# faustomorales/keras-ocr

Hardware: AMD Instinct MI355X
Metric: images/sec end-to-end Pipeline.recognize() @768x768 (higher is better)
Workload: dtype f32 (fp32 operands as 2 fp16 pieces [F(4,3) / head layers] or 3 bf16 pieces [1x1, dilated], 3 / 6 MFMA products, fp32 accumulate; fp32-class error vs fp64: tests/test_conv_gpu.py)

## Files before the change

keras_ocr_amd/csrc/elementwise.hip:

```cpp
#include "split_common.h"
#include <algorithm>

struct EwParams {
  const float* in;
  float* out;
  int N, Hi, Wi, Ho, Wo, C4;
  int in_cs, in_co, out_cs, out_co;
  float sy, sx;
  int row_off;
  int Wov;
};

__global__ void maxpool2x2_kernel(EwParams p) {
  const size_t total = (size_t)p.N * p.Ho * p.Wo * p.C4;
  for (size_t i = blockIdx.x * (size_t)blockDim.x + threadIdx.x; i < total;
       i += (size_t)gridDim.x * blockDim.x) {
    const int c4 = i % p.C4;
    size_t t = i / p.C4;
    const int ox = t % p.Wo;
    t /= p.Wo;
    const int oy = t % p.Ho;
    const int n = t / p.Ho;
    const size_t o = (((size_t)n * p.Ho + oy) * p.Wo + ox) * p.out_cs + p.out_co + c4 * 4;
    if (ox >= p.Wov) {
      *reinterpret_cast<float4*>(p.out + o) = float4{0.f, 0.f, 0.f, 0.f};
      continue;
    }
    const size_t base = (((size_t)n * p.Hi + 2 * oy + p.row_off) * p.Wi + 2 * ox) * p.in_cs + p.in_co + c4 * 4;
    const float4 a = *reinterpret_cast<const float4*>(p.in + base);
    const float4 b = *reinterpret_cast<const float4*>(p.in + base + p.in_cs);
    const float4 c = *reinterpret_cast<const float4*>(p.in + base + (size_t)p.Wi * p.in_cs);
    const float4 d = *reinterpret_cast<const float4*>(p.in + base + (size_t)p.Wi * p.in_cs + p.in_cs);
    float4 r;
    r.x = fmaxf(fmaxf(a.x, b.x), fmaxf(c.x, d.x));
    r.y = fmaxf(fmaxf(a.y, b.y), fmaxf(c.y, d.y));
    r.z = fmaxf(fmaxf(a.z, b.z), fmaxf(c.z, d.z));
    r.w = fmaxf(fmaxf(a.w, b.w), fmaxf(c.w, d.w));
    *reinterpret_cast<float4*>(p.out + o) = r;
  }
}

__global__ void maxpool3x3s1_kernel(EwParams p) {
  const size_t total = (size_t)p.N * p.Ho * p.Wo * p.C4;
  for (size_t i = blockIdx.x * (size_t)blockDim.x + threadIdx.x; i < total;
       i += (size_t)gridDim.x * blockDim.x) {
    const int c4 = i % p.C4;
    size_t t = i / p.C4;
    const int ox = t % p.Wo;
    t /= p.Wo;
    const int oy = t % p.Ho;
    const int n = t / p.Ho;
    float4 r = make_float4(-INFINITY, -INFINITY, -INFINITY, -INFINITY);
    for (int dy = -1; dy <= 1; ++dy) {
      const int iy = oy + dy;
      if (iy < 0 || iy >= p.Hi) continue;
      for (int dx = -1; dx <= 1; ++dx) {
        const int ix = ox + dx;
        if (ix < 0 || ix >= p.Wi) continue;
        const float4 v = *reinterpret_cast<const float4*>(
            p.in + (((size_t)n * p.Hi + iy) * p.Wi + ix) * p.in_cs + p.in_co + c4 * 4);
        r.x = fmaxf(r.x, v.x);
        r.y = fmaxf(r.y, v.y);
        r.z = fmaxf(r.z, v.z);
        r.w = fmaxf(r.w, v.w);
      }
    }
    const size_t o = (((size_t)n * p.Ho + oy) * p.Wo + ox) * p.out_cs + p.out_co + c4 * 4;
    *reinterpret_cast<float4*>(p.out + o) = r;
  }
}

__global__ void resize_bilinear_kernel(EwParams p) {
  const size_t total = (size_t)p.N * p.Ho * p.Wo * p.C4;
  for (size_t i = blockIdx.x * (size_t)blockDim.x + threadIdx.x; i < total;
       i += (size_t)gridDim.x * blockDim.x) {
    const int c4 = i % p.C4;
    size_t t = i / p.C4;
    const int ox = t % p.Wo;
    t /= p.Wo;
    const int oy = t % p.Ho;
    const int n = t / p.Ho;
    const float fy = ((float)oy + 0.5f) * p.sy - 0.5f;
    const float fx = ((float)ox + 0.5f) * p.sx - 0.5f;
    const float fly = floorf(fy), flx = floorf(fx);
    const int y0 = max((int)fly, 0), y1 = min((int)ceilf(fy), p.Hi - 1);
    const int x0 = max((int)flx, 0), x1 = min((int)ceilf(fx), p.Wi - 1);
    const float yl = fy - fly, xl = fx - flx, yk = 1.f - yl, xk = 1.f - xl;
    const size_t rb = (size_t)n * p.Hi;
    const float* b0 = p.in + ((rb + y0) * p.Wi) * p.in_cs + p.in_co + c4 * 4;
    const float* b1 = p.in + ((rb + y1) * p.Wi) * p.in_cs + p.in_co + c4 * 4;
    const float4 tl = *reinterpret_cast<const float4*>(b0 + (size_t)x0 * p.in_cs);
    const float4 tr = *reinterpret_cast<const float4*>(b0 + (size_t)x1 * p.in_cs);
    const float4 bl = *reinterpret_cast<const float4*>(b1 + (size_t)x0 * p.in_cs);
    const float4 br = *reinterpret_cast<const float4*>(b1 + (size_t)x1 * p.in_cs);
    float4 r;
    {
      const float top = tl.x * xk + tr.x * xl, bot = bl.x * xk + br.x * xl;
      r.x = top * yk + bot * yl;
    }
    {
      const float top = tl.y * xk + tr.y * xl, bot = bl.y * xk + br.y * xl;
      r.y = top * yk + bot * yl;
    }
    {
      const float top = tl.z * xk + tr.z * xl, bot = bl.z * xk + br.z * xl;
      r.z = top * yk + bot * yl;
    }
    {
      const float top = tl.w * xk + tr.w * xl, bot = bl.w * xk + br.w * xl;
      r.w = top * yk + bot * yl;
    }
    const size_t o = (((size_t)n * p.Ho + oy) * p.Wo + ox) * p.out_cs + p.out_co + c4 * 4;
    *reinterpret_cast<float4*>(p.out + o) = r;
  }
}

__global__ void copy_channels_kernel(EwParams p) {
  const size_t total = (size_t)p.N * p.Ho * p.Wo * p.C4;
  for (size_t i = blockIdx.x * (size_t)blockDim.x + threadIdx.x; i < total;
       i += (size_t)gridDim.x * blockDim.x) {
    const int c4 = i % p.C4;
    const size_t px = i / p.C4;
    *reinterpret_cast<float4*>(p.out + px * p.out_cs + p.out_co + c4 * 4) =
        *reinterpret_cast<const float4*>(p.in + px * p.in_cs + p.in_co + c4 * 4);
  }
}

static int check_vec(kocr_ctx* ctx, const Tensor& in, const Tensor& out, const char* what) {
  if (in.C != out.C || in.N != out.N) KOCR_FAIL(ctx, KOCR_EINVAL, std::string(what) + ": shape mismatch");
  if (in.C % 4 || in.cs % 4 || in.co % 4 || out.cs % 4 || out.co % 4)
    KOCR_FAIL(ctx, KOCR_EINVAL, std::string(what) + ": channels must be multiples of 4");
  return KOCR_OK;
}

static EwParams make_params(const Tensor& in, const Tensor& out) {
  EwParams p;
  p.in = in.p;
  p.out = out.p;
  p.N = in.N;
  p.Hi = in.H;
  p.Wi = in.W;
  p.Ho = out.H;
  p.Wo = out.W;
  p.C4 = in.C / 4;
  p.in_cs = in.cs;
  p.in_co = in.co;
  p.out_cs = out.cs;
  p.out_co = out.co;
  p.sy = p.sx = 1.f;
  p.row_off = 0;
  p.Wov = out.W;
  return p;
}

static dim3 ew_grid(size_t total) {
  size_t b = (total + 255) / 256;
  if (b > 256 * 16) b = 256 * 16;
  if (b == 0) b = 1;
  return dim3((unsigned)b);
}

int launch_maxpool2x2(kocr_ctx* ctx, const Tensor& in, const Tensor& out, int row_off) {
  KOCR_TRY(check_vec(ctx, in, out, "maxpool2x2"));
  if (out.H != (in.H - row_off) / 2 || out.wv() != in.wv() / 2) KOCR_FAIL(ctx, KOCR_EINVAL, "maxpool2x2: bad output size");
  EwParams p = make_params(in, out);
  p.row_off = row_off;
  p.Wov = out.wv();
  const size_t total = out.pixels() * p.C4;
  if (!total) return KOCR_OK;
  {
    ProfScope ps(ctx, "maxpool2x2", 0, 4.0 * (in.pixels() + out.pixels()) * in.C);
    hipLaunchKernelGGL(maxpool2x2_kernel, ew_grid(total), dim3(256), 0, ctx->stream, p);
    KOCR_HIP(ctx, hipGetLastError());
  }
  if (out.amax) {
    if (in.amax) return launch_amax_copy(ctx, in.amax, out.amax, out.N);
    return launch_absmax(ctx, out, out.amax);
  }
  return KOCR_OK;
}

int launch_maxpool3x3s1(kocr_ctx* ctx, const Tensor& in, const Tensor& out) {
  KOCR_TRY(check_vec(ctx, in, out, "maxpool3x3s1"));
  if (out.H != in.H || out.W != in.W) KOCR_FAIL(ctx, KOCR_EINVAL, "maxpool3x3s1: bad output size");
  EwParams p = make_params(in, out);
  const size_t total = out.pixels() * p.C4;
  if (!total) return KOCR_OK;
  {
    ProfScope ps(ctx, "maxpool3x3s1", 0, 4.0 * (in.pixels() + out.pixels()) * in.C);
    hipLaunchKernelGGL(maxpool3x3s1_kernel, ew_grid(total), dim3(256), 0, ctx->stream, p);
    KOCR_HIP(ctx, hipGetLastError());
  }
  if (out.amax) {
    if (in.amax) return launch_amax_copy(ctx, in.amax, out.amax, out.N);
    return launch_absmax(ctx, out, out.amax);
  }
  return KOCR_OK;
}

int launch_resize_bilinear(kocr_ctx* ctx, const Tensor& in, const Tensor& out) {
  KOCR_TRY(check_vec(ctx, in, out, "resize_bilinear"));
  EwParams p = make_params(in, out);
  p.sy = (float)in.H / (float)out.H;
  p.sx = (float)in.W / (float)out.W;
  const size_t total = out.pixels() * p.C4;
  if (!total) return KOCR_OK;
  {
    ProfScope ps(ctx, "resize_bilinear", 0, 4.0 * (in.pixels() + out.pixels()) * in.C);
    hipLaunchKernelGGL(resize_bilinear_kernel, ew_grid(total), dim3(256), 0, ctx->stream, p);
    KOCR_HIP(ctx, hipGetLastError());
  }
  if (out.amax) {
    if (in.amax) return launch_amax_copy(ctx, in.amax, out.amax, out.N);
    return launch_absmax(ctx, out, out.amax);
  }
  return KOCR_OK;
}

int launch_copy_channels(kocr_ctx* ctx, const Tensor& in, const Tensor& out) {
  KOCR_TRY(check_vec(ctx, in, out, "copy_channels"));
  if (out.H != in.H || out.W != in.W) KOCR_FAIL(ctx, KOCR_EINVAL, "copy_channels: bad output size");
  EwParams p = make_params(in, out);
  const size_t total = out.pixels() * p.C4;
  if (!total) return KOCR_OK;
  ProfScope ps(ctx, "copy_channels", 0, 8.0 * out.pixels() * in.C);
  hipLaunchKernelGGL(copy_channels_kernel, ew_grid(total), dim3(256), 0, ctx->stream, p);
  KOCR_HIP(ctx, hipGetLastError());
  return KOCR_OK;
}

struct HeadTailParams {
  const float* in;
  float* out;
  const float* w6;
  const float* a6;
  const float* b6;
  const float* w8;
  const float* a8;
  const float* b8;
  int ld6, ld8, in_cs, in_co, relu6;
  size_t P;
};

__global__ __launch_bounds__(256) void head_tail_kernel(HeadTailParams p) {
  __shared__ float s_w6[16][16], s_a6[16], s_b6[16], s_w8[16][2], s_a8[2], s_b8[2];
  const int tid = threadIdx.x;
  s_w6[tid >> 4][tid & 15] = p.w6[(tid >> 4) * p.ld6 + (tid & 15)];
  if (tid < 16) {
    s_a6[tid] = p.a6[tid];
    s_b6[tid] = p.b6[tid];
    s_w8[tid][0] = p.w8[tid * p.ld8 + 0];
    s_w8[tid][1] = p.w8[tid * p.ld8 + 1];
  }
  if (tid < 2) {
    s_a8[tid] = p.a8[tid];
    s_b8[tid] = p.b8[tid];
  }
  __syncthreads();
  typedef float v4f __attribute__((ext_vector_type(4)));
  typedef float v2f __attribute__((ext_vector_type(2)));
  for (size_t i = blockIdx.x * (size_t)blockDim.x + tid; i < p.P; i += (size_t)gridDim.x * blockDim.x) {
    const float* src = p.in + i * p.in_cs + p.in_co;
    float x[16];
#pragma unroll
    for (int q = 0; q < 4; ++q) {
      const v4f v = *reinterpret_cast<const v4f*>(src + 4 * q);
      x[4 * q + 0] = v.x;
      x[4 * q + 1] = v.y;
      x[4 * q + 2] = v.z;
      x[4 * q + 3] = v.w;
    }
    float y0 = 0.f, y1 = 0.f;
#pragma unroll
    for (int o = 0; o < 16; ++o) {
      float h = 0.f;
#pragma unroll
      for (int c = 0; c < 16; ++c) h = fmaf(x[c], s_w6[c][o], h);
      h = h * s_a6[o] + s_b6[o];
      if (p.relu6) h = fmaxf(h, 0.f);
      y0 = fmaf(h, s_w8[o][0], y0);
      y1 = fmaf(h, s_w8[o][1], y1);
    }
    *reinterpret_cast<v2f*>(p.out + 2 * i) = v2f{y0 * s_a8[0] + s_b8[0], y1 * s_a8[1] + s_b8[1]};
  }
}

int launch_head_tail(kocr_ctx* ctx, const ConvLayer& L6, const ConvLayer& L8, const Tensor& in, float* d_heat) {
  if (L6.Cin != 16 || L6.Cout != 16 || L6.KH != 1 || L8.Cin != 16 || L8.Cout != 2 || L8.KH != 1 || L8.relu ||
      L6.d_post_a || L8.d_post_a || !L6.tap_inner || !L8.tap_inner || in.C != 16 || in.cs % 4 || in.co % 4)
    KOCR_FAIL(ctx, KOCR_EINVAL, "head_tail: unexpected layer shapes");
  HeadTailParams p;
  p.in = in.p;
  p.out = d_heat;
  p.w6 = L6.d_w;
  p.a6 = L6.d_pre_a;
  p.b6 = L6.d_pre_b;
  p.w8 = L8.d_w;
  p.a8 = L8.d_pre_a;
  p.b8 = L8.d_pre_b;
  p.ld6 = L6.Cout_pad;
  p.ld8 = L8.Cout_pad;
  p.in_cs = in.cs;
  p.in_co = in.co;
  p.relu6 = L6.relu;
  p.P = in.pixels();
  if (!p.P) return KOCR_OK;
  const double flops = 2.0 * (double)p.P * (16 * 16 + 16 * 2);
  ProfScope ps(ctx, "conv_head_tail", flops, (double)p.P * (64 + 8));
  hipLaunchKernelGGL(head_tail_kernel, ew_grid(p.P), dim3(256), 0, ctx->stream, p);
  KOCR_HIP(ctx, hipGetLastError());
  return KOCR_OK;
}

__global__ __launch_bounds__(256) void absmax_kernel(const float* in, size_t img_pixels, int C4, int cs, int co, unsigned* slots) {
  typedef float v4f __attribute__((ext_vector_type(4)));
  float m = 0.f;
  const size_t total = img_pixels * C4;
  const float* base = in + (size_t)blockIdx.y * img_pixels * cs;
  for (size_t i = blockIdx.x * (size_t)blockDim.x + threadIdx.x; i < total; i += (size_t)gridDim.x * blockDim.x) {
    const size_t px = i / C4;
    const int c4 = (int)(i - px * C4);
    const v4f v = *reinterpret_cast<const v4f*>(base + px * cs + co + 4 * c4);
    m = fmaxf(m, fmaxf(fmaxf(fabsf(v.x), fabsf(v.y)), fmaxf(fabsf(v.z), fabsf(v.w))));
  }
  kocr_amax_update(slots + blockIdx.y, m);
}

__global__ void amax_copy_kernel(const unsigned* from, unsigned* to, int n) {
  const int i = blockIdx.x * blockDim.x + threadIdx.x;
  if (i < n) atomicMax(to + i, from[i]);
}

int launch_absmax(kocr_ctx* ctx, const Tensor& t, unsigned* slots) {
  if (t.C % 4 || t.cs % 4 || t.co % 4 || ((uintptr_t)t.p & 15)) KOCR_FAIL(ctx, KOCR_EINVAL, "absmax: unaligned tensor");
  const size_t total = (size_t)t.H * t.W * (t.C / 4);
  if (!total || !t.N) return KOCR_OK;
  ProfScope ps(ctx, "absmax", 0, 4.0 * t.pixels() * t.C);
  size_t b = (total + 4095) / 4096;
  const size_t cap = std::max<size_t>(1, 4096 / (size_t)t.N);
  if (b > cap) b = cap;
  constexpr int NCHUNK = 32768;
  for (int n0 = 0; n0 < t.N; n0 += NCHUNK) {
    const int nn = std::min(NCHUNK, t.N - n0);
    hipLaunchKernelGGL(absmax_kernel, dim3((unsigned)b, (unsigned)nn), dim3(256), 0, ctx->stream,
                       t.p + (size_t)n0 * t.H * t.W * t.cs, (size_t)t.H * t.W, t.C / 4, t.cs, t.co, slots + n0);
    KOCR_HIP(ctx, hipGetLastError());
  }
  return KOCR_OK;
}

__global__ __launch_bounds__(256) void range_stats_kernel(const float* in, int H, int W, int C4, int cs, int co, const unsigned* slots,
                                                          int cells, int cellW, int top, unsigned long long* cnt, double* sums, int n0) {
  typedef float v4f __attribute__((ext_vector_type(4)));
  const int n = n0 + blockIdx.y;
  const size_t img_pixels = (size_t)H * W, total = img_pixels * C4;
  const float* base = in + (size_t)n * img_pixels * cs;
  unsigned long long c0 = 0, c1 = 0, c2 = 0;
  double s0 = 0, s1 = 0;
  for (size_t i = blockIdx.x * (size_t)blockDim.x + threadIdx.x; i < total; i += (size_t)gridDim.x * blockDim.x) {
    const size_t px = i / C4;
    const int c4 = (int)(i - px * C4);
    const int slot = cells ? n * cells + (int)((px % W) / cellW) : n;
    const int e = kocr_scale_exp(slots + slot, top);
    const float sc = kocr_pow2(e);
    const v4f v = *reinterpret_cast<const v4f*>(base + px * cs + co + 4 * c4);
#pragma unroll
    for (int k = 0; k < 4; ++k) {
      const float a = fabsf(v[k]), s = a * sc;
      if (a > 0.f) {
        ++c0;
        s0 += a;
        if (s < 0.0625f) {
          ++c1;
          s1 += a;
        }
        if (s < 6.103515625e-05f) ++c2;
      }
    }
  }
  atomicAdd(cnt + 0, c0);
  atomicAdd(cnt + 1, c1);
  atomicAdd(cnt + 2, c2);
  atomicAdd(sums + 0, s0);
  atomicAdd(sums + 1, s1);
}

int launch_range_stats(kocr_ctx* ctx, const std::string& name, const Tensor& t, const unsigned* slots, int top) {
  if (!ctx->range_on || !slots || t.C % 4 || t.cs % 4 || t.co % 4 || !t.pixels()) return KOCR_OK;
  if (!ctx->d_range) KOCR_FAIL(ctx, KOCR_EINVAL, "range statistics: call kocr_range_stats_enable first");
  unsigned long long* cnt = (unsigned long long*)ctx->d_range;
  double* sums = (double*)((char*)ctx->d_range + 32);
  KOCR_HIP(ctx, hipMemsetAsync(ctx->d_range, 0, 64, ctx->stream));
  size_t b = ((size_t)t.H * t.W * (t.C / 4) + 4095) / 4096;
  if (b > 64) b = 64;
  constexpr int NCHUNK = 32768;
  for (int n0 = 0; n0 < t.N; n0 += NCHUNK) {
    hipLaunchKernelGGL(range_stats_kernel, dim3((unsigned)b, (unsigned)std::min(NCHUNK, t.N - n0)), dim3(256), 0, ctx->stream, t.p, t.H,
                       t.W, t.C / 4, t.cs, t.co, slots, t.cells(), t.cellW ? t.cellW : 1, top, cnt, sums, n0);
    KOCR_HIP(ctx, hipGetLastError());
  }
  unsigned long long hc[4];
  double hs[4];
  KOCR_HIP(ctx, hipMemcpyAsync(hc, cnt, 32, hipMemcpyDeviceToHost, ctx->stream));
  KOCR_HIP(ctx, hipMemcpyAsync(hs, sums, 32, hipMemcpyDeviceToHost, ctx->stream));
  KOCR_HIP(ctx, hipStreamSynchronize(ctx->stream));
  RangeRow& r = ctx->range[name];
  r.launches += 1;
  r.elements += (double)t.pixels() * t.C;
  r.nonzero += (double)hc[0];
  r.below_m4 += (double)hc[1];
  r.below_m14 += (double)hc[2];
  r.sum_abs += hs[0];
  r.sum_abs_below_m4 += hs[1];
  return KOCR_OK;
}

int launch_amax_copy(kocr_ctx* ctx, const unsigned* from, unsigned* to, int n) {
  if (!from || !to || from == to || n <= 0) return KOCR_OK;
  hipLaunchKernelGGL(amax_copy_kernel, dim3((n + 255) / 256), dim3(256), 0, ctx->stream, from, to, n);
  KOCR_HIP(ctx, hipGetLastError());
  return KOCR_OK;
}
```

keras_ocr_amd/csrc/imgproc.hip:

```cpp
#include "common.h"
#include <cmath>

struct ResizeTables {
  int* xi0;
  int* xi1;
  int* xa0;
  int* xa1;
  int* yi0;
  int* yi1;
  int* yb0;
  int* yb1;
};

namespace {
void axis_tables(int src, int dst, bool horizontal, std::vector<int>& i0, std::vector<int>& i1, std::vector<int>& c0,
                 std::vector<int>& c1) {
  const double scale = (double)src / (double)dst;
  i0.resize(dst);
  i1.resize(dst);
  c0.resize(dst);
  c1.resize(dst);
  for (int d = 0; d < dst; ++d) {
    float f = (float)((d + 0.5) * scale - 0.5);
    int s = (int)std::floor(f);
    f = f - (float)s;
    if (horizontal) {
      if (s < 0) {
        f = 0.f;
        s = 0;
      }
      if (s >= src - 1) {
        f = 0.f;
        s = src - 1;
      }
    }
    c1[d] = (int)std::nearbyint(f * 2048.f);
    c0[d] = (int)std::nearbyint((1.f - f) * 2048.f);
    i0[d] = std::min(std::max(s, 0), src - 1);
    i1[d] = std::min(std::max(s + 1, 0), src - 1);
  }
}
}

__global__ void resize_pad_kernel(const uint8_t* __restrict__ src, int sh, int sw, size_t src_img_stride,
                                  uint8_t* __restrict__ dst, int dh, int dw, int Hmax, int Wmax, int cval, ResizeTables t) {
  const int n = blockIdx.z, y = blockIdx.y;
  const int x = blockIdx.x * blockDim.x + threadIdx.x;
  if (x >= Wmax) return;
  uint8_t* o = dst + (((size_t)n * Hmax + y) * Wmax + x) * 3;
  if (y >= dh || x >= dw) {
    o[0] = o[1] = o[2] = (uint8_t)cval;
    return;
  }
  const uint8_t* im = src + (size_t)n * src_img_stride;
  const int x0 = t.xi0[x], x1 = t.xi1[x], a0 = t.xa0[x], a1 = t.xa1[x];
  const int y0 = t.yi0[y], y1 = t.yi1[y], b0 = t.yb0[y], b1 = t.yb1[y];
  const uint8_t* r0 = im + (size_t)y0 * sw * 3;
  const uint8_t* r1 = im + (size_t)y1 * sw * 3;
#pragma unroll
  for (int c = 0; c < 3; ++c) {
    const int S0 = r0[x0 * 3 + c] * a0 + r0[x1 * 3 + c] * a1;
    const int S1 = r1[x0 * 3 + c] * a0 + r1[x1 * 3 + c] * a1;
    const int v = (((b0 * (S0 >> 4)) >> 16) + ((b1 * (S1 >> 4)) >> 16) + 2) >> 2;
    o[c] = (uint8_t)min(max(v, 0), 255);
  }
}

int launch_resize_pad(kocr_ctx* ctx, const uint8_t* d_src, int n, int sh, int sw, uint8_t* d_dst, int dh, int dw,
                      int Hmax, int Wmax, int cval, Arena& tab_arena) {
  if (n <= 0) return KOCR_OK;
  if (dh <= 0 || dw <= 0 || dh > Hmax || dw > Wmax || sh <= 0 || sw <= 0)
    KOCR_FAIL(ctx, KOCR_EINVAL, "resize_pad: bad sizes");
  std::vector<int> tb[8];
  axis_tables(sw, dw, true, tb[0], tb[1], tb[2], tb[3]);
  axis_tables(sh, dh, false, tb[4], tb[5], tb[6], tb[7]);
  std::vector<int> flat;
  for (auto& v : tb) flat.insert(flat.end(), v.begin(), v.end());
  int* d_tab = (int*)arena_alloc(tab_arena, flat.size() * sizeof(int));
  if (!d_tab) KOCR_FAIL(ctx, KOCR_ENOMEM, "resize_pad: table arena exhausted");
  KOCR_HIP(ctx, hipMemcpyAsync(d_tab, flat.data(), flat.size() * sizeof(int), hipMemcpyHostToDevice, ctx->stream));
  KOCR_HIP(ctx, hipStreamSynchronize(ctx->stream));
  ResizeTables t;
  t.xi0 = d_tab;
  t.xi1 = t.xi0 + dw;
  t.xa0 = t.xi1 + dw;
  t.xa1 = t.xa0 + dw;
  t.yi0 = t.xa1 + dw;
  t.yi1 = t.yi0 + dh;
  t.yb0 = t.yi1 + dh;
  t.yb1 = t.yb0 + dh;
  ProfScope ps(ctx, "resize_pad", 0, 3.0 * n * ((double)sh * sw + (double)Hmax * Wmax));
  hipLaunchKernelGGL(resize_pad_kernel, dim3((Wmax + 255) / 256, Hmax, n), dim3(256), 0, ctx->stream, d_src, sh, sw,
                     (size_t)sh * sw * 3, d_dst, dh, dw, Hmax, Wmax, cval, t);
  KOCR_HIP(ctx, hipGetLastError());
  return KOCR_OK;
}


struct ResizeTablesF {
  int* xi0;
  int* xi1;
  float* xa;
  int* yi0;
  int* yi1;
  float* ya;
};

__global__ void resize_pad_f32_kernel(const float* __restrict__ src, int sh, int sw, int C, float* __restrict__ dst, int dh, int dw,
                                      int Hmax, int Wmax, float cval, ResizeTablesF t) {
  const int n = blockIdx.z, y = blockIdx.y;
  const int x = blockIdx.x * blockDim.x + threadIdx.x;
  if (x >= Wmax) return;
  float* o = dst + (((size_t)n * Hmax + y) * Wmax + x) * C;
  if (y >= dh || x >= dw) {
    for (int c = 0; c < C; ++c) o[c] = cval;
    return;
  }
  const float* im = src + (size_t)n * sh * sw * C;
  const int x0 = t.xi0[x], x1 = t.xi1[x], y0 = t.yi0[y], y1 = t.yi1[y];
  const float ax = t.xa[x], ay = t.ya[y];
  const float* r0 = im + (size_t)y0 * sw * C;
  const float* r1 = im + (size_t)y1 * sw * C;
  for (int c = 0; c < C; ++c) {
    const float h0 = r0[x0 * C + c] * (1.f - ax) + r0[x1 * C + c] * ax;
    const float h1 = r1[x0 * C + c] * (1.f - ax) + r1[x1 * C + c] * ax;
    o[c] = h0 * (1.f - ay) + h1 * ay;
  }
}

int launch_resize_pad_f32(kocr_ctx* ctx, const float* d_src, int n, int sh, int sw, int C, float* d_dst, int dh, int dw, int Hmax,
                          int Wmax, float cval, Arena& tab_arena) {
  if (n <= 0) return KOCR_OK;
  if (dh <= 0 || dw <= 0 || dh > Hmax || dw > Wmax || sh <= 0 || sw <= 0 || C <= 0) KOCR_FAIL(ctx, KOCR_EINVAL, "resize_pad_f32: bad sizes");
  std::vector<int> flat((size_t)3 * (dw + dh));
  auto taps = [&](int dst_n, int src_n, int* i0, int* i1, float* a) {
    for (int d = 0; d < dst_n; ++d) {
      const double f = (d + 0.5) * ((double)src_n / (double)dst_n) - 0.5;
      long s = (long)std::floor(f);
      float w = (float)(f - (double)s);
      if (s < 0 || s >= src_n - 1) w = 0.f;
      const long c0 = std::min<long>(std::max<long>(s, 0), src_n - 1);
      i0[d] = (int)c0;
      i1[d] = (int)std::min<long>(c0 + 1, src_n - 1);
      a[d] = w;
    }
  };
  int* xi0 = flat.data();
  int* xi1 = xi0 + dw;
  float* xa = reinterpret_cast<float*>(xi1 + dw);
  int* yi0 = reinterpret_cast<int*>(xa + dw);
  int* yi1 = yi0 + dh;
  float* ya = reinterpret_cast<float*>(yi1 + dh);
  taps(dw, sw, xi0, xi1, xa);
  taps(dh, sh, yi0, yi1, ya);
  int* d_tab = (int*)arena_alloc(tab_arena, flat.size() * sizeof(int));
  if (!d_tab) KOCR_FAIL(ctx, KOCR_ENOMEM, "resize_pad_f32: table arena exhausted");
  KOCR_HIP(ctx, hipMemcpyAsync(d_tab, flat.data(), flat.size() * sizeof(int), hipMemcpyHostToDevice, ctx->stream));
  KOCR_HIP(ctx, hipStreamSynchronize(ctx->stream));
  ResizeTablesF t;
  t.xi0 = d_tab;
  t.xi1 = t.xi0 + dw;
  t.xa = reinterpret_cast<float*>(t.xi1 + dw);
  t.yi0 = reinterpret_cast<int*>(t.xa + dw);
  t.yi1 = t.yi0 + dh;
  t.ya = reinterpret_cast<float*>(t.yi1 + dh);
  ProfScope ps(ctx, "resize_pad_f32", 0, 4.0 * C * n * ((double)sh * sw + (double)Hmax * Wmax));
  hipLaunchKernelGGL(resize_pad_f32_kernel, dim3((Wmax + 255) / 256, Hmax, n), dim3(256), 0, ctx->stream, d_src, sh, sw, C, d_dst, dh, dw,
                     Hmax, Wmax, cval, t);
  KOCR_HIP(ctx, hipGetLastError());
  return KOCR_OK;
}
```

Before: 263.6.

## Rewrite maxpool3x3, head tail loads and uint8 resize with row reuse and staging

The 3x3 stride-1 maxpool now has each thread own two output columns across an 8-row strip, keeping a sliding window of three input rows in registers instead of re-reading nine taps per output. The head tail kernel stages each wave's 64 pixels through shared memory so the global loads are coalesced before the per-pixel 16x16 and 16x2 matmuls. The uint8 resize-pad kernel is rewritten to stage source rows in LDS with double-buffered prefetch, handle four pixels per thread, extract taps with alignbyte, and write packed 32-bit words. These are three unrelated elementwise kernels, each small in end-to-end time, and the new code adds barriers and complexity, including edge-case handling for image borders.

```diff
diff --git a/keras_ocr_amd/csrc/elementwise.hip b/keras_ocr_amd/csrc/elementwise.hip
--- a/keras_ocr_amd/csrc/elementwise.hip
+++ b/keras_ocr_amd/csrc/elementwise.hip
@@ -40,33 +40,70 @@
   }
 }
 
-__global__ void maxpool3x3s1_kernel(EwParams p) {
-  const size_t total = (size_t)p.N * p.Ho * p.Wo * p.C4;
-  for (size_t i = blockIdx.x * (size_t)blockDim.x + threadIdx.x; i < total;
-       i += (size_t)gridDim.x * blockDim.x) {
-    const int c4 = i % p.C4;
-    size_t t = i / p.C4;
-    const int ox = t % p.Wo;
-    t /= p.Wo;
-    const int oy = t % p.Ho;
-    const int n = t / p.Ho;
-    float4 r = make_float4(-INFINITY, -INFINITY, -INFINITY, -INFINITY);
-    for (int dy = -1; dy <= 1; ++dy) {
-      const int iy = oy + dy;
-      if (iy < 0 || iy >= p.Hi) continue;
-      for (int dx = -1; dx <= 1; ++dx) {
-        const int ix = ox + dx;
-        if (ix < 0 || ix >= p.Wi) continue;
-        const float4 v = *reinterpret_cast<const float4*>(
-            p.in + (((size_t)n * p.Hi + iy) * p.Wi + ix) * p.in_cs + p.in_co + c4 * 4);
-        r.x = fmaxf(r.x, v.x);
-        r.y = fmaxf(r.y, v.y);
-        r.z = fmaxf(r.z, v.z);
-        r.w = fmaxf(r.w, v.w);
+constexpr int MP_ROWS = 8;
+
+struct MpRow {
+  float4 v[4];
+};
+
+__device__ __forceinline__ void mp_fold(float4& r, const float4& v) {
+  r.x = fmaxf(r.x, v.x);
+  r.y = fmaxf(r.y, v.y);
+  r.z = fmaxf(r.z, v.z);
+  r.w = fmaxf(r.w, v.w);
+}
+
+__global__ __launch_bounds__(256) void maxpool3x3s1_kernel(EwParams p, unsigned xblocks, unsigned strips) {
+  const unsigned xb = blockIdx.x % xblocks, bt = blockIdx.x / xblocks;
+  const unsigned strip = bt % strips, n = bt / strips;
+  const unsigned item = xb * 256u + threadIdx.x;
+  const unsigned xp = item / (unsigned)p.C4;
+  const int c4 = (int)(item - xp * (unsigned)p.C4);
+  const int x0 = 2 * (int)xp, y0 = (int)strip * MP_ROWS;
+  if (x0 >= p.Wo) return;
+  const float4 ninf = make_float4(-INFINITY, -INFINITY, -INFINITY, -INFINITY);
+  bool colok[4];
+  size_t icol[4];
+#pragma unroll
+  for (int j = 0; j < 4; ++j) {
+    const int ix = x0 - 1 + j;
+    colok[j] = ix >= 0 && ix < p.Wi;
+    icol[j] = (size_t)min(max(ix, 0), p.Wi - 1) * p.in_cs;
+  }
+  const float* ibase = p.in + (size_t)n * p.Hi * p.Wi * p.in_cs + p.in_co + c4 * 4;
+  float* obase = p.out + ((size_t)n * p.Ho * p.Wo + (size_t)x0) * p.out_cs + p.out_co + c4 * 4;
+  const size_t irow = (size_t)p.Wi * p.in_cs, orow = (size_t)p.Wo * p.out_cs;
+  MpRow a, b, c;
+#pragma unroll
+  for (int k = 0; k < MP_ROWS + 2; ++k) {
+    const int iy = y0 - 1 + k;
+    if (iy > p.Hi) break;
+    const bool rowok = iy >= 0 && iy < p.Hi;
+    const float* irp = ibase + (size_t)min(max(iy, 0), p.Hi - 1) * irow;
+#pragma unroll
+    for (int j = 0; j < 4; ++j) {
+      const float4 v = *reinterpret_cast<const float4*>(irp + icol[j]);
+      c.v[j] = rowok && colok[j] ? v : ninf;
+    }
+    if (k >= 2) {
+      const int oy = iy - 1;
+      if (oy < p.Ho) {
+#pragma unroll
+        for (int q = 0; q < 2; ++q) {
+          if (x0 + q >= p.Wo) continue;
+          float4 r = ninf;
+#pragma unroll
+          for (int dx = 0; dx < 3; ++dx) mp_fold(r, a.v[q + dx]);
+#pragma unroll
+          for (int dx = 0; dx < 3; ++dx) mp_fold(r, b.v[q + dx]);
+#pragma unroll
+          for (int dx = 0; dx < 3; ++dx) mp_fold(r, c.v[q + dx]);
+          *reinterpret_cast<float4*>(obase + (size_t)oy * orow + (size_t)q * p.out_cs) = r;
+        }
       }
     }
-    const size_t o = (((size_t)n * p.Ho + oy) * p.Wo + ox) * p.out_cs + p.out_co + c4 * 4;
-    *reinterpret_cast<float4*>(p.out + o) = r;
+    a = b;
+    b = c;
   }
 }
 
@@ -187,8 +224,11 @@
   const size_t total = out.pixels() * p.C4;
   if (!total) return KOCR_OK;
   {
+    const size_t xblocks = ((size_t)((out.W + 1) / 2) * p.C4 + 255) / 256, strips = (out.H + MP_ROWS - 1) / MP_ROWS;
+    const size_t blocks = (size_t)out.N * strips * xblocks;
+    if (blocks > 0x7fffffffu) KOCR_FAIL(ctx, KOCR_EINVAL, "maxpool3x3s1: tensor too large for one launch");
     ProfScope ps(ctx, "maxpool3x3s1", 0, 4.0 * (in.pixels() + out.pixels()) * in.C);
-    hipLaunchKernelGGL(maxpool3x3s1_kernel, ew_grid(total), dim3(256), 0, ctx->stream, p);
+    hipLaunchKernelGGL(maxpool3x3s1_kernel, dim3((unsigned)blocks), dim3(256), 0, ctx->stream, p, (unsigned)xblocks, (unsigned)strips);
     KOCR_HIP(ctx, hipGetLastError());
   }
   if (out.amax) {
@@ -242,6 +282,8 @@
   size_t P;
 };
 
+constexpr int HT_LD = 20;
+
 __global__ __launch_bounds__(256) void head_tail_kernel(HeadTailParams p) {
   __shared__ float s_w6[16][16], s_a6[16], s_b6[16], s_w8[16][2], s_a8[2], s_b8[2];
   const int tid = threadIdx.x;
@@ -259,17 +301,30 @@
   __syncthreads();
   typedef float v4f __attribute__((ext_vector_type(4)));
   typedef float v2f __attribute__((ext_vector_type(2)));
-  for (size_t i = blockIdx.x * (size_t)blockDim.x + tid; i < p.P; i += (size_t)gridDim.x * blockDim.x) {
-    const float* src = p.in + i * p.in_cs + p.in_co;
+  __shared__ __attribute__((aligned(16))) float s_x[4][64][HT_LD];
+  const int lane = tid & 63, wave = tid >> 6;
+  for (size_t base = blockIdx.x * (size_t)256; base < p.P; base += (size_t)gridDim.x * 256) {
+    const size_t wbase = base + 64 * wave;
+#pragma unroll
+    for (int q = 0; q < 4; ++q) {
+      const int px = 16 * q + (lane >> 2);
+      if (wbase + px < p.P)
+        *reinterpret_cast<v4f*>(&s_x[wave][px][4 * (lane & 3)]) =
+            *reinterpret_cast<const v4f*>(p.in + (wbase + px) * p.in_cs + p.in_co + 4 * (lane & 3));
+    }
+    __syncthreads();
+    const size_t i = base + tid;
     float x[16];
 #pragma unroll
     for (int q = 0; q < 4; ++q) {
-      const v4f v = *reinterpret_cast<const v4f*>(src + 4 * q);
+      const v4f v = *reinterpret_cast<const v4f*>(&s_x[wave][lane][4 * q]);
       x[4 * q + 0] = v.x;
       x[4 * q + 1] = v.y;
       x[4 * q + 2] = v.z;
       x[4 * q + 3] = v.w;
     }
+    __syncthreads();
+    if (i >= p.P) continue;
     float y0 = 0.f, y1 = 0.f;
 #pragma unroll
     for (int o = 0; o < 16; ++o) {
diff --git a/keras_ocr_amd/csrc/imgproc.hip b/keras_ocr_amd/csrc/imgproc.hip
--- a/keras_ocr_amd/csrc/imgproc.hip
+++ b/keras_ocr_amd/csrc/imgproc.hip
@@ -42,27 +42,135 @@
 }
 }
 
-__global__ void resize_pad_kernel(const uint8_t* __restrict__ src, int sh, int sw, size_t src_img_stride,
-                                  uint8_t* __restrict__ dst, int dh, int dw, int Hmax, int Wmax, int cval, ResizeTables t) {
-  const int n = blockIdx.z, y = blockIdx.y;
-  const int x = blockIdx.x * blockDim.x + threadIdx.x;
-  if (x >= Wmax) return;
-  uint8_t* o = dst + (((size_t)n * Hmax + y) * Wmax + x) * 3;
-  if (y >= dh || x >= dw) {
-    o[0] = o[1] = o[2] = (uint8_t)cval;
-    return;
-  }
+constexpr int RP_PX = 4, RP_STAGE = 4096, RP_ROWS = 8;
+constexpr int RP_SPAN = RP_PX * 256 + 3;
+
+struct RpRow {
+  uint8_t* orow;
+  const uint8_t* src[2];
+  int xb;
+  int off[2], words[2];
+  int lo, b0, b1;
+  bool inside, staged;
+};
+
+__global__ __launch_bounds__(256) void resize_pad_kernel(const uint8_t* __restrict__ src, int sh, int sw, size_t src_img_stride,
+                                                         uint8_t* __restrict__ dst, int dh, int dw, int Hmax, int Wmax, int cval,
+                                                         ResizeTables t) {
+  __shared__ uint32_t s_row[2][RP_STAGE / 4 + 1];
+  __shared__ int s_xt[4][RP_SPAN], s_yt[4][RP_ROWS];
+  const int n = blockIdx.z, tid = threadIdx.x, yb = (int)blockIdx.y * RP_ROWS;
+  const int X0 = RP_PX * 256 * (int)blockIdx.x - RP_PX;
+  const int tx0 = max(X0, 0), tx1 = min(X0 + RP_SPAN, dw);
+  for (int i = tid; i < tx1 - tx0; i += 256) {
+    s_xt[0][i] = t.xi0[tx0 + i];
+    s_xt[1][i] = t.xi1[tx0 + i];
+    s_xt[2][i] = t.xa0[tx0 + i];
+    s_xt[3][i] = t.xa1[tx0 + i];
+  }
+  if (tid < RP_ROWS && yb + tid < dh) {
+    s_yt[0][tid] = t.yi0[yb + tid];
+    s_yt[1][tid] = t.yi1[yb + tid];
+    s_yt[2][tid] = t.yb0[yb + tid];
+    s_yt[3][tid] = t.yb1[yb + tid];
+  }
+  __syncthreads();
   const uint8_t* im = src + (size_t)n * src_img_stride;
-  const int x0 = t.xi0[x], x1 = t.xi1[x], a0 = t.xa0[x], a1 = t.xa1[x];
-  const int y0 = t.yi0[y], y1 = t.yi1[y], b0 = t.yb0[y], b1 = t.yb1[y];
-  const uint8_t* r0 = im + (size_t)y0 * sw * 3;
-  const uint8_t* r1 = im + (size_t)y1 * sw * 3;
-#pragma unroll
-  for (int c = 0; c < 3; ++c) {
-    const int S0 = r0[x0 * 3 + c] * a0 + r0[x1 * 3 + c] * a1;
-    const int S1 = r1[x0 * 3 + c] * a0 + r1[x1 * 3 + c] * a1;
-    const int v = (((b0 * (S0 >> 4)) >> 16) + ((b1 * (S1 >> 4)) >> 16) + 2) >> 2;
-    o[c] = (uint8_t)min(max(v, 0), 255);
+  auto plan = [&](int k) -> RpRow {
+    RpRow R;
+    const int y = yb + k;
+    R.orow = dst + ((size_t)n * Hmax + y) * Wmax * 3;
+    R.xb = X0 + (int)((uintptr_t)R.orow & 3);
+    const int xs = max(R.xb, 0), xe = min(min(R.xb + RP_PX * 256, Wmax), dw);
+    R.inside = y < dh && xs < xe;
+    R.staged = false;
+    R.src[0] = R.src[1] = im;
+    R.off[0] = R.off[1] = R.words[0] = R.words[1] = R.lo = R.b0 = R.b1 = 0;
+    if (R.inside) {
+      R.src[0] = im + (size_t)s_yt[0][k] * sw * 3;
+      R.src[1] = im + (size_t)s_yt[1][k] * sw * 3;
+      R.b0 = s_yt[2][k];
+      R.b1 = s_yt[3][k];
+      R.lo = s_xt[0][xs - tx0];
+      const int hi = s_xt[1][xe - 1 - tx0], nb = 3 * (hi - R.lo + 1);
+#pragma unroll
+      for (int i = 0; i < 2; ++i) {
+        R.off[i] = (int)((uintptr_t)(R.src[i] + 3 * (size_t)R.lo) & 3);
+        R.words[i] = (R.off[i] + nb + 3) / 4;
+      }
+      R.staged = max(R.words[0], R.words[1]) <= RP_STAGE / 4;
+    }
+    return R;
+  };
+  uint32_t w[2][RP_STAGE / 4 / 256];
+  auto fetch = [&](const RpRow& R) {
+    if (!R.staged) return;
+#pragma unroll
+    for (int i = 0; i < 2; ++i) {
+      const uint32_t* from = reinterpret_cast<const uint32_t*>(R.src[i] + 3 * (size_t)R.lo - R.off[i]);
+#pragma unroll
+      for (int q = 0; q < RP_STAGE / 4 / 256; ++q)
+        if (tid + 256 * q < R.words[i]) w[i][q] = from[tid + 256 * q];
+    }
+  };
+  auto stash = [&](const RpRow& R) {
+    if (!R.staged) return;
+#pragma unroll
+    for (int i = 0; i < 2; ++i)
+#pragma unroll
+      for (int q = 0; q < RP_STAGE / 4 / 256; ++q)
+        if (tid + 256 * q < R.words[i]) s_row[i][tid + 256 * q] = w[i][q];
+  };
+  RpRow cur = plan(0);
+  fetch(cur);
+  for (int k = 0; k < RP_ROWS && yb + k < Hmax; ++k) {
+    stash(cur);
+    __syncthreads();
+    RpRow nxt = cur;
+    if (k + 1 < RP_ROWS && yb + k + 1 < Hmax) {
+      nxt = plan(k + 1);
+      fetch(nxt);
+    }
+    auto tap = [&](int i, int xi) -> uint32_t {
+      if (cur.staged) {
+        const int o = cur.off[i] + 3 * (xi - cur.lo);
+        return __builtin_amdgcn_alignbyte(s_row[i][(o >> 2) + 1], s_row[i][o >> 2], (uint32_t)(o & 3));
+      }
+      const uint8_t* p = cur.src[i] + 3 * (size_t)xi;
+      return (uint32_t)p[0] | ((uint32_t)p[1] << 8) | ((uint32_t)p[2] << 16);
+    };
+    auto pixel = [&](int x) -> uint32_t {
+      if (!cur.inside || x >= dw) return (uint32_t)(cval & 255) * 0x010101u;
+      const int x0 = s_xt[0][x - tx0], x1 = s_xt[1][x - tx0], a0 = s_xt[2][x - tx0], a1 = s_xt[3][x - tx0];
+      const uint32_t p00 = tap(0, x0), p01 = tap(0, x1), p10 = tap(1, x0), p11 = tap(1, x1);
+      uint32_t out = 0;
+#pragma unroll
+      for (int c = 0; c < 3; ++c) {
+        const int S0 = __mul24((int)((p00 >> (8 * c)) & 255), a0) + __mul24((int)((p01 >> (8 * c)) & 255), a1);
+        const int S1 = __mul24((int)((p10 >> (8 * c)) & 255), a0) + __mul24((int)((p11 >> (8 * c)) & 255), a1);
+        const int v = ((__mul24(cur.b0, S0 >> 4) >> 16) + (__mul24(cur.b1, S1 >> 4) >> 16) + 2) >> 2;
+        out |= (uint32_t)min(max(v, 0), 255) << (8 * c);
+      }
+      return out;
+    };
+    const int x = cur.xb + RP_PX * tid;
+    if (x >= 0 && x + RP_PX <= Wmax) {
+      const uint32_t p0 = pixel(x), p1 = pixel(x + 1), p2 = pixel(x + 2), p3 = pixel(x + 3);
+      uint32_t* o = reinterpret_cast<uint32_t*>(cur.orow + 3 * (size_t)x);
+      o[0] = p0 | (p1 << 24);
+      o[1] = (p1 >> 8) | (p2 << 16);
+      o[2] = (p2 >> 16) | (p3 << 8);
+    } else {
+      for (int j = max(x, 0); j < min(x + RP_PX, Wmax); ++j) {
+        const uint32_t p = pixel(j);
+        uint8_t* o = cur.orow + 3 * (size_t)j;
+        o[0] = (uint8_t)p;
+        o[1] = (uint8_t)(p >> 8);
+        o[2] = (uint8_t)(p >> 16);
+      }
+    }
+    __syncthreads();
+    cur = nxt;
   }
 }
 
@@ -90,7 +198,8 @@
   t.yb0 = t.yi1 + dh;
   t.yb1 = t.yb0 + dh;
   ProfScope ps(ctx, "resize_pad", 0, 3.0 * n * ((double)sh * sw + (double)Hmax * Wmax));
-  hipLaunchKernelGGL(resize_pad_kernel, dim3((Wmax + 255) / 256, Hmax, n), dim3(256), 0, ctx->stream, d_src, sh, sw,
+  const int groups = (Wmax + RP_PX - 1) / RP_PX + 1;
+  hipLaunchKernelGGL(resize_pad_kernel, dim3((groups + 255) / 256, (Hmax + RP_ROWS - 1) / RP_ROWS, n), dim3(256), 0, ctx->stream, d_src, sh, sw,
                      (size_t)sh * sw * 3, d_dst, dh, dw, Hmax, Wmax, cval, t);
   KOCR_HIP(ctx, hipGetLastError());
   return KOCR_OK;
```

Measured after the change: 264.5 (median of 6 runs). Within noise of the previous version (+0.4%).
